# gersteinlab/LESSeq

Hardware: AMD Instinct MI355X
Metric: MRF reads/sec through count+solve (higher is better)
Workload: dtype int32 coordinates / u64 counters (count), f64 (EM); 1 GPU; BASELINE configs[2]: 100M synthetic 100bp reads over 50k mixed events (SE/RI/A5SS/A3SS/MXE/AFE/ALE/T3), 24 chromosomes; events=50000

## Files before the change

include/lesseq_hip_dev.h:

```cpp
#ifndef LESSEQ_HIP_DEV_H
#define LESSEQ_HIP_DEV_H

#include <stdint.h>
#include "lesseq_hip.h"

#ifdef __cplusplus
extern "C" {
#endif

int lsq_debug_counters(lsq_ctx *c, unsigned long long *out16);
int lsq_debug_wg_trace(lsq_ctx *c, unsigned long long *out, unsigned long long cap, unsigned long long *n, unsigned long long *n_workers);

int lsq_debug_slot_offsets(lsq_ctx *c, int method, unsigned long long *out, unsigned long long n);
int lsq_debug_plan_shares(const unsigned long long *slot_off, const unsigned char *packed, const unsigned long long *n1, const unsigned long long *n2,
                          const unsigned *look1, const unsigned *look2, unsigned long long n_buckets, unsigned long long grid,
                          const double *costs4, int weighted, int snap, unsigned long long *cuts);
int lsq_debug_offsets(lsq_ctx *c, int method, int which, unsigned long long *out, unsigned long long cap, unsigned long long *n);

int lsq_debug_set_em_order(lsq_ctx *c, const uint32_t *order, unsigned n_small_places, unsigned n_places);

int lsq_debug_last_em_launch(lsq_ctx *c, unsigned out[8]);

int lsq_debug_stream_read_rate(lsq_ctx *c, unsigned long long bytes, double *gb_per_s);

int lsq_debug_throw(int kind);

int lsq_debug_last_parse_paths(const lsq_ctx *c, unsigned *tiles_handed, unsigned *lines_listed, unsigned *all_slow);

int lsq_debug_bgzf_inflate(lsq_ctx *c, const void *bytes, uint64_t len, void *out, uint64_t cap, uint64_t *n);

int lsq_debug_bgzf_crc32(lsq_ctx *c, const void *bytes, uint64_t len, uint32_t *crc, uint64_t cap, uint64_t *n);

// ... 9 lines not shown
```

lesseq_amd/csrc/lsq_count.hip:

```cpp
#include "lsq_device.hpp"
#include <hip/hip_ext.h>

namespace {

#ifndef LSQ_COUNT_BLOCK
#define LSQ_COUNT_BLOCK 256
#endif
constexpr int COUNT_BLOCK = LSQ_COUNT_BLOCK;
constexpr unsigned long long BASES_MASK = (1ull << 40) - 1;

#ifdef LSQ_DEV
#define ABL(args, bits) ((((args).ablate) & (bits)) != 0u)
#else
#define ABL(args, bits) false
#endif


struct CountArgs {
	const BucketDesc *buckets;
	const unsigned char *images;
	const TieRec *ties;
	const unsigned char *strand_rank;
	const char *read_names; const unsigned long long *read_name_off;
	const char *gene_names; const unsigned *gene_name_off;
	unsigned n_buckets;
	unsigned ablate;
	unsigned tables_lds_bytes;
	const void *p1; const unsigned char *p1_strand; const unsigned *p1_line;
	const void *p2; const unsigned char *p2_strand; const unsigned *p2_line;
	unsigned compact;
	const unsigned *pn_blk_off; const unsigned *pn_nblk; const int2 *pn_se; const unsigned char *pn_strand; const unsigned *pn_line; const unsigned *pn_bucket;
	const unsigned long long *p1_off, *p2_off, *pn_off, *slot_off;
	const lsq::VisitRec *visits;
	const unsigned *wg_first;
	const unsigned long long *wg_cut;
	const lsq::WgPlan *wg_plan;
	unsigned long long *wg_trace;
	unsigned long long total_slots;
	unsigned long long n_pn;
	unsigned n_workers;
	unsigned long long *cnt, *bases;
	struct ExcEntry *exc;
	unsigned *exc_count;
	unsigned exc_cap;
	unsigned long long *dbg;
// ... 604 lines not shown
	};
	if (ww0 < ww1) fetch(ww0);
	for (unsigned wt = ww0; wt < ww1; wt += WAVES * TILE) {
		uint4 cur[SW];
#pragma unroll
		for (int k = 0; k < SW; ++k) cur[k] = nxt[k];
		if (wt + WAVES * TILE < ww1) fetch(wt + WAVES * TILE);
		do_step(cur, wt);
	}
	if (R.live() && !ABL(A, 32u)) walk_parked<NB>(C, R, true);
}


template <int NR>
__device__ inline void stream_pool1_compact(FastCtx &C, const uint4 *bins, const uint4 *cells, const uint4 *cellx, const unsigned n_cells, const BucketDesc &d,
                                            const CountArgs &A, uint4 *queue, const void *pool, const unsigned long long g0, const unsigned long long g1) {
	static_assert(NR == 4 || NR == 8, "one or two 16-byte words of four compact records");
	static_assert((unsigned)NR <= P1_GROUP_PAD, "a lane's records of a step lie in one cell group");
	constexpr int CW = NR / 4;
	constexpr unsigned TILE = 64u * NR;
	C.pool = 0u;
	C.slot0 = g0;
	global_words src = (global_words)pool;
	const unsigned lane = threadIdx.x & 63u, wave = (unsigned)__builtin_amdgcn_readfirstlane((int)(threadIdx.x >> 6));
	const unsigned long long R0 = g0 & ~(unsigned long long)(NR - 1);
	const unsigned n = (unsigned)(g1 - R0), first_rel = (unsigned)(g0 - R0), n_rel = (unsigned)(g1 - g0);
	const unsigned last_word = (n - 1u) >> 2;
	const int base = d.lo - lsq::COMPACT_BIAS;
	uint4 nxt[CW];
	auto fetch = [&](const unsigned t) {
#pragma unroll
// ... 37 lines not shown
#pragma unroll
			for (int j = 0; j < NR; ++j) {
				const unsigned len = rec[j] >> lsq::COMPACT_OFF_BITS;
				const int e = (int)(rec[j] & lsq::COMPACT_OFF_MASK) + (int)len;
				unsigned p = len | (min(len, 1u) << 24);
				if (!decltype(whole_step)::value) {
					const unsigned idx = t + lane * (unsigned)NR + (unsigned)j;
					p = (idx < n && idx - first_rel < n_rel) ? p : 0u;
				}
				accN += p;
				accA += e <= e1 ? p : 0u;
				if (!decltype(one_threshold)::value) accL += e <= e2 ? p : 0u;
			}
			if (decltype(one_threshold)::value) accL = accA;
		};
		if (__all(e1 == e2) && !ABL(A, 8388608u)) { if (interior) decide(std::true_type{}, std::true_type{}); else decide(std::false_type{}, std::true_type{}); }
		else { if (interior) decide(std::true_type{}, std::false_type{}); else decide(std::false_type{}, std::false_type{}); }
		const unsigned s1 = cx.x & 0xFFFFu, s2 = cx.x >> 16;
		if (!ABL(A, (1u | 16384u))) {
			const unsigned acc2 = both ? accL : accL - accA;
			if (accA && s1 != CELL_NONE) atomicAdd(&C.hist[s1], ((unsigned long long)(accA >> 24) << 40) | (accA & 0xFFFFFFu));
			if (acc2 && s2 != CELL_NONE) atomicAdd(&C.hist[s2], ((unsigned long long)(acc2 >> 24) << 40) | (acc2 & 0xFFFFFFu));
		} else asm volatile("" ::"v"(accA), "v"(accL));
		const bool lane_open = (accN >> 24) != ((both ? accA : accL) >> 24);
		if (ABL(A, 256u)) {
			const bool any_open = __any(lane_open);
			if (lane == 0) { atomicAdd(&A.dbg[12], 1ull); atomicAdd(&A.dbg[11], any_open ? 1ull : 0ull); }
		}
		if (__any(lane_open) && !ABL(A, 17u | 524288u)) {
#pragma unroll
			for (int h = 0; h < NR; h += 2) {
// ... 16 lines not shown
					if (ABL(A, 256u) && op) { atomicAdd(&A.dbg[5 + (has ? (both ? 2 : 1) : 0)], 1ull); atomicAdd(&A.dbg[0], 1ull); }
				}
				R.push2(open, lane, en[0], en[1]);
				if (R.live() >= 64u) {
					if (!ABL(A, 32u)) walk_parked<1, false>(C, R, false, base);
					else R.head = R.tail;
				}
			}
		}
	}
	if (R.live() && !ABL(A, 32u)) walk_parked<1, false>(C, R, true, base);
}

template <int NR>
__device__ inline void stream_pool2_compact(FastCtx &C, const uint4 *bins, const uint4 *cells, const uint4 *cellx, const unsigned n_cells, const BucketDesc &d,
                                            const CountArgs &A, uint4 *queue, const void *pool, const unsigned long long g0, const unsigned long long g1) {
	static_assert((NR == 2 || NR == 4 || NR == 8) && (unsigned)NR <= P2_GROUP_PAD, "whole 16-byte words of two compact records, inside one junction group");
	constexpr int CW = NR / 2;
	constexpr unsigned TILE = 64u * NR;
	C.pool = 1u;
	C.slot0 = g0;
	global_words src = (global_words)pool;
	const unsigned lane = threadIdx.x & 63u, wave = (unsigned)__builtin_amdgcn_readfirstlane((int)(threadIdx.x >> 6));
	const unsigned long long R0 = g0 & ~(unsigned long long)(NR - 1);
	const unsigned n = (unsigned)(g1 - R0), first_rel = (unsigned)(g0 - R0), n_rel = (unsigned)(g1 - g0);
	const unsigned last_word = (n - 1u) >> 1;
	const int base = d.lo - lsq::COMPACT_BIAS;
	uint4 nxt[CW];
	auto fetch = [&](const unsigned t) {
#pragma unroll
		for (int cq = 0; cq < CW; ++cq) {
// ... 76 lines not shown
		};
		bool none[NR];
#pragma unroll
		for (int j = 0; j < NR; ++j) none[j] = false;
		if (any_plain) {
#pragma unroll
			for (int j = 0; j < NR; ++j) none[j] = !junction && nothing(ra[j], rb[j]);
		}
		bool park[NR];
		park[0] = in0 && len1 != 0u && !(J || Jb || S || drop || none[0]) && !ABL(A, 17u | 1048576u);
		if (ABL(A, 256u) && park[0]) atomicAdd(&A.dbg[8 + (v1 ? 1 : 0)], 1ull);
		unsigned nA = (in0 && J && slotA != CELL_NONE) ? 1u : 0u, sA = nA ? total : 0u, nB = (in0 && Jb && slotB != CELL_NONE) ? 1u : 0u, sB = nB ? total : 0u;
		const int lim = junction ? end2 - rd.y : -1, limb = junction ? end2b - rd.y : -1;
		bool any_park = park[0];
		const bool any_b = __any(limb > lim) || ABL(A, 8388608u);
#pragma unroll
		for (int j = 1; j < NR; ++j) {
			const unsigned l1 = ra[j] >> lsq::COMPACT_OFF_BITS, l2 = rb[j] >> lsq::COMPACT_OFF_BITS;
			const int reach = (int)(rb[j] & lsq::COMPACT_OFF_MASK) + (int)l2;
			bool in = l1 != 0u;
			if (!interior) { const unsigned idx = idx0 + (unsigned)j; in = in && idx < n && idx - first_rel < n_rel; }
			const bool sameA = in && reach <= lim;
			bool sameB = false;
			const bool cA = sameA && slotA != CELL_NONE;
			nA += cA ? 1u : 0u; sA += cA ? l1 + l2 : 0u;
			if (any_b) {
				sameB = in && reach > lim && reach <= limb;
				const bool cB = sameB && slotB != CELL_NONE;
				nB += cB ? 1u : 0u; sB += cB ? l1 + l2 : 0u;
			}
			park[j] = in && !(sameA || sameB || none[j]) && !ABL(A, 17u | 1048576u | 2097152u);
			if (ABL(A, 256u) && park[j]) atomicAdd(&A.dbg[junction ? 14 : 13], 1ull);
			any_park = any_park || park[j];
		}
		if (!ABL(A, 1u)) {
			if (addS) atomicAdd(&C.hist[sa], (1ull << 40) | len1);
			if (nA) atomicAdd(&C.hist[slotA], ((unsigned long long)nA << 40) | sA);
			if (nB) atomicAdd(&C.hist[slotB], ((unsigned long long)nB << 40) | sB);
		} else asm volatile("" ::"v"(nA), "v"(sA), "v"(nB), "v"(sB));
		if (__any(any_park)) {
			const unsigned hint0 = v1 ? (cx1.w | PARK_ONE_EVENT) : evf;
#pragma unroll
			for (int h = 0; h < NR; h += 2) {
				const uint4 qa = make_uint4(ra[h], rb[h], h == 0 ? hint0 : PARK_EVENT_UNKNOWN, rel0 + (unsigned)h);
				const uint4 qb = make_uint4(ra[h + 1], rb[h + 1], PARK_EVENT_UNKNOWN, rel0 + (unsigned)h + 1u);
				if (ABL(A, 256u)) atomicAdd(&A.dbg[1], (park[h] ? 1ull : 0ull) + (park[h + 1] ? 1ull : 0ull));
				R.push2((park[h] ? 1u : 0u) | (park[h + 1] ? 2u : 0u), lane, qa, qb);
				if (R.live() >= 64u) {
					if (!ABL(A, 32u)) walk_parked<2, true>(C, R, false, base);
// ... 102 lines not shown
	const unsigned long long s_begin = plan->s_begin, s_end = plan->s_end;
	if (s_begin >= s_end) return;
	if (ABL(A, 4096u)) return;
	const_visit vr = &plan->first;
	unsigned b = vr->b;
	bool first_visit = true;
	while (b < A.n_buckets) {
		const unsigned long long bs = vr->bs;
		if (bs >= s_end) break;
		BucketDesc d;
		d.img_off = vr->d.img_off; d.img_bytes = vr->d.img_bytes; d.n_events = vr->d.n_events; d.n_bins = vr->d.n_bins; d.lo = vr->d.lo; d.shift = vr->d.shift;
		d.ev_off = vr->d.ev_off; d.seg_off = vr->d.seg_off; d.iso_off = vr->d.iso_off; d.hist_off = vr->d.hist_off; d.n_cls = vr->d.n_cls; d.cls_base = vr->d.cls_base;
		d.ev_base = vr->d.ev_base; d.chrom_id = vr->d.chrom_id; d.kind = vr->d.kind; d.hi = vr->d.hi;
		const unsigned long long be = vr->be, p1o = vr->p1o, n1 = vr->p1n, p2o = vr->p2o, n2 = vr->p2n;
		const unsigned next = vr->next;
		unsigned char *buf = lds;
		if (!first_visit) __syncthreads();
		first_visit = false;
		{
			global_words src = (global_words)(A.images + d.img_off);
			uint4 *dst = reinterpret_cast<uint4 *>(buf);
			for (unsigned i = tid; i < d.img_bytes / 16; i += COUNT_BLOCK) { const u32x4 t = src[i]; dst[i] = make_uint4(t.x, t.y, t.z, t.w); }
			unsigned long long *h = reinterpret_cast<unsigned long long *>(buf + d.hist_off);
			for (unsigned i = tid; i < HIST_REPLICAS * (d.n_cls | 1u); i += COUNT_BLOCK) h[i] = 0;
		}
		__syncthreads();
		if (ABL(A, 8192u)) return;
		const uint4 *bins = reinterpret_cast<const uint4 *>(buf);
		const uint4 *cells = reinterpret_cast<const uint4 *>(buf + d.seg_off);
		const unsigned n_cells = d.iso_off & 0xFFFFu;
		const uint4 *cellx = reinterpret_cast<const uint4 *>(buf + d.seg_off + 16u * (d.iso_off >> 16));
		FastCtx C;
		C.bins = bins; C.lo = d.lo; C.shift = d.shift; C.n_bins = d.n_bins;
		C.recs = reinterpret_cast<const uint4 *>(buf + d.ev_off);
		C.hist = reinterpret_cast<unsigned long long *>(buf + d.hist_off) + (tid & (HIST_REPLICAS - 1u)) * (d.n_cls | 1u);
		C.n_events = d.n_events; C.bucket = b;
		C.slot0 = 0; C.pool = 0;
		C.exc = A.exc; C.exc_count = A.exc_count; C.exc_cap = A.exc_cap; C.ablate = A.ablate; C.dbg = A.dbg;
		C.trace = (ABL(A, 4194304u) && A.wg_trace) ? A.wg_trace + 4u * blockIdx.x : nullptr;
		const unsigned long long l0 = (s_begin > bs ? s_begin : bs) - bs;
		const unsigned long long l1 = (s_end < be ? s_end : be) - bs;
		if (l0 < n1 && !ABL(A, 1024u)) {
			if constexpr (COMPACT) stream_pool1_compact<2 * P1W>(C, bins, cells, cellx, n_cells, d, A, wave_queue, A.p1, p1o + l0, p1o + (l1 < n1 ? l1 : n1));
			else stream_pool_wide<2>(C, bins, cells, cellx, n_cells, d, A, wave_queue, reinterpret_cast<const uint4 *>(A.p1), p1o + l0, p1o + (l1 < n1 ? l1 : n1));
		}
		if (l1 > n1 && l0 < n1 + n2 && !ABL(A, 2048u)) {
			const unsigned long long q0 = p2o + ((l0 > n1 ? l0 : n1) - n1), q1 = p2o + ((l1 < n1 + n2 ? l1 : n1 + n2) - n1);
			if constexpr (COMPACT) stream_pool2_compact<(P1W == 4 ? LSQ_P2_COMPACT_WORDS_W5 : LSQ_P2_COMPACT_WORDS)>(C, bins, cells, cellx, n_cells, d, A, wave_queue, A.p2, q0, q1);
			else stream_pool_wide<1>(C, bins, cells, cellx, n_cells, d, A, wave_queue, reinterpret_cast<const uint4 *>(A.p2), q0, q1);
		}
		__syncthreads();
		for (unsigned i = tid; i < d.n_cls; i += COUNT_BLOCK) {
			const unsigned long long *h0 = reinterpret_cast<const unsigned long long *>(buf + d.hist_off) + i;
			unsigned long long v = 0;
#pragma unroll
			for (unsigned r = 0; r < HIST_REPLICAS; ++r) v += h0[r * (d.n_cls | 1u)];
			if (v && !ABL(A, 4u)) {
				atomicAdd(&A.cnt[d.cls_base + i], v >> 40);
				atomicAdd(&A.bases[d.cls_base + i], v & BASES_MASK);
			}
		}
		if (be >= s_end) break;
		b = next;
// ... 297 lines not shown
				if ((rc = mr.wg_plan.upload(plan.data(), plan.size(), st))) return rc;
				HIP_TRY(hipStreamSynchronize(st));
			}
			HIP_TRY(hipStreamSynchronize(st));
			mr.wg_grid = grid;
		}
		CountArgs A{};
		A.buckets = c->buckets.p; A.images = c->images.p; A.ties = c->ties.p; A.strand_rank = c->strand_rank.p;
		A.wg_first = mr.wg_first.p; A.wg_cut = mr.wg_cut.p; A.wg_plan = mr.wg_plan.p; A.visits = mr.visits.p;
		A.read_names = mr.named ? mr.names.p : nullptr; A.read_name_off = mr.named ? mr.name_off.p : nullptr;
		A.gene_names = c->gene_names.p; A.gene_name_off = c->gene_name_off.p;
		A.n_buckets = (unsigned)E.buckets.size();
		A.tables_lds_bytes = tables_bytes;
		A.ablate = c->dev_ablate;
		A.compact = mr.compact ? 1u : 0u;
		A.p1 = mr.p1.p; A.p1_strand = mr.p1_strand.p; A.p1_line = mr.p1_line.p;
		A.p2 = mr.p2.p; A.p2_strand = mr.p2_strand.p; A.p2_line = mr.p2_line.p;
		A.pn_blk_off = mr.pn_blk_off.p; A.pn_nblk = mr.pn_nblk.p; A.pn_se = reinterpret_cast<const int2 *>(mr.pn_se.p);
		A.pn_strand = mr.pn_strand.p; A.pn_line = mr.pn_line.p; A.pn_bucket = mr.pn_bucket.p;
		A.p1_off = mr.p1_off.p; A.p2_off = mr.p2_off.p; A.pn_off = mr.pn_off.p; A.slot_off = mr.slot_off.p;
		A.total_slots = mr.total_slots;
		A.cnt = c->cnt.p + (size_t)m * n_cls; A.bases = c->bases.p + (size_t)m * n_cls;
		A.exc = mr.exc.p + (size_t)set * mr.exc_cap; A.exc_count = c->exc_count.p + 2 * m; A.exc_cap = (unsigned)mr.exc_cap;
		A.dbg = c->dbg.p; A.bar = c->dbg.p + 16 + m;
		A.wg_trace = nullptr;
		const unsigned long long n_pn = mr.pn_strand.n;
		A.n_pn = n_pn;
		const unsigned workers_per_cu = 2;
		A.n_workers = (unsigned)std::min<unsigned long long>((n_pn + COUNT_BLOCK - 1) / COUNT_BLOCK, (unsigned long long)c->n_cu * workers_per_cu);
#ifdef LSQ_DEV
// ... 136 lines not shown
```

lesseq_amd/csrc/lsq_device.hip:

```cpp
#include "lsq_device.hpp"
#include <chrono>
#include <thread>

namespace lsq {

int upload_strand_ranks(lsq_ctx *c) {
	const auto &names = c->E->strands.names;
	if (names.size() > 256) return fail(LSQ_E_RANGE, "more than 256 distinct strand strings");
	std::vector<int> order(names.size());
	std::iota(order.begin(), order.end(), 0);
	std::sort(order.begin(), order.end(), [&](int a, int b) { return names[a] < names[b]; });
	std::vector<uint8_t> rank(256, 0);
	for (size_t r = 0; r < order.size(); ++r) rank[order[r]] = (uint8_t)r;
	int rc = c->strand_rank.upload(rank.data(), 256, c->stream);
	if (rc) return rc;
	HIP_TRY(hipStreamSynchronize(c->stream));
	return LSQ_OK;
}

static hipError_t wait_for_stream(hipStream_t s) {
	const auto t0 = std::chrono::steady_clock::now();
	for (;;) {
		const hipError_t e = hipStreamQuery(s);
		if (e != hipErrorNotReady) return e;
// ... 817 lines not shown
	} else if (n == "sam_min_mapq") {
		if (!(value >= 0 && value <= 256)) return fail(LSQ_E_ARG, "sam_min_mapq must lie in 0..256");
		c->opt_sam_min_mapq = (unsigned)value;
	} else if (n == "bam_verify") {
		if (!(value == 0 || value == 1)) return fail(LSQ_E_ARG, "bam_verify must be 0 or 1");
		c->opt_bam_verify = value == 1;
	} else if (n == "compact_pools") {
		c->opt_compact_pools = value != 0;
	} else if (n == "workgroups_per_cu") {
		if (!(value >= -1 && value <= 32)) return fail(LSQ_E_ARG, "workgroups_per_cu must lie in -1..32 (-1 = automatic, 0 = as many as fit)");
		c->opt_wg_per_cu = (int)value;
		c->occ_lds_bytes = 0;
	} else if (n == "reads_per_look") {
		if (!(value == 0 || value == 4 || value == 8)) return fail(LSQ_E_ARG, "reads_per_look must be 0 (automatic), 4 or 8");
		c->opt_reads_per_look = (int)value;
	} else if (n == "count_streams") {
		{ int rc = sync_all(c); if (rc) return rc; }
		c->opt_two_count_streams = value >= 2;
	} else if (n == "em_flat_min_events") {
		if (!(value >= 0 && value <= 4e9)) return fail(LSQ_E_ARG, "em_flat_min_events must lie in 0..4e9");
		c->em.opt_flat_min = (unsigned)value;
	} else if (n == "em_closed_form") {
		{ int rc = sync_all(c); if (rc) return rc; }
		c->em.opt_closed = value != 0;
	} else if (n == "em_quad_cap") {
		if (value < 0 || value > 1e6) return fail(LSQ_E_ARG, "em_quad_cap out of range");
		c->em.opt_quad_cap = (unsigned)value;
	} else if (n == "em_regroup") {
		c->em.opt_regroup = value != 0;
		for (EmLane &l : c->em.lane) l.order_valid = false;
// ... 41 lines not shown
```

lesseq_amd/csrc/lsq_device.hpp:

```cpp
#pragma once
#include <hip/hip_runtime.h>

#include <algorithm>
#include <cmath>
#include <cstring>
#include <memory>
#include <numeric>
#include <string>
#include <thread>
#include <type_traits>
#include <vector>

#include "lsq_internal.hpp"

using namespace lsq;

#define HIP_TRY(expr)                                                                          \
	do {                                                                                       \
		hipError_t _e = (expr);                                                                \
		if (_e != hipSuccess) return fail(LSQ_E_DEVICE, "%s: %s", #expr, hipGetErrorString(_e)); \
	} while (0)


#ifndef LSQ_P1_PAD
// ... 60 lines not shown
}

struct RouteChrom {
	unsigned loc_first, loc_nb;
	int loc_base;
	unsigned cov0, cov1, clu0, clu1;
	unsigned pad;
};
static_assert(sizeof(RouteChrom) == 32, "RouteChrom is staged in LDS as two 16-byte words");

struct VisitRec {
	BucketDesc d;
	unsigned long long bs, be;
	unsigned long long p1o, p1n, p2o, p2n;
	unsigned b, next;
	unsigned pad[2];
};
static_assert(sizeof(VisitRec) == 128, "VisitRec is read as 32 dwords");
struct WgPlan {
	unsigned long long s_begin, s_end;
	VisitRec first;
};
static_assert(sizeof(WgPlan) == 144, "WgPlan layout");

struct IngestPass {
	const char *name = nullptr;
	hipEvent_t ev[2] = {nullptr, nullptr};
	unsigned long long bytes = 0;
	float ms = 0;
	bool clocked = false;
};
// ... 76 lines not shown
	hipStream_t stream_em2[2] = {nullptr, nullptr};
	hipStream_t stream_count2[2] = {nullptr, nullptr};
	bool opt_two_count_streams = true;
	int opt_wg_per_cu = -1;
	hipEvent_t ev_counted2[2] = {nullptr, nullptr}, ev_mark2[2] = {nullptr, nullptr};
	bool mark_recorded2[2] = {false, false};
	int flip = 0;
	size_t counters_per_set = 0;
	hipEvent_t ev0 = nullptr, ev1 = nullptr, ev2 = nullptr, ev3 = nullptr;
	hipEvent_t evt0 = nullptr, evt1 = nullptr;
	hipEvent_t evf0[LSQ_MAX_METHODS] = {}, evf1[LSQ_MAX_METHODS] = {};
	int fast_launched = 0;
	int occ_p1w = 0;
	int opt_reads_per_look = 0;
	unsigned last_reads_per_look = 4, last_wg_per_cu = 0;
	unsigned occ_lds_bytes = 0; int occ_blocks = 0;
	bool time_events = false;
	bool count_timed = false, solve_timed = false;
	lsq_events *E = nullptr;
	DevBuf<BucketDesc> buckets;
	DevBuf<uint8_t> images, strand_rank, dK;
	DevBuf<TieRec> ties;
	DevBuf<uint32_t> cls_base, iso_base, gene_name_off;
	DevBuf<char> gene_names;
	DevBuf<uint32_t> pack_cls, pack_iso, pack_ev;
	EmState em;
	DevBuf<double> G, theta2[2], logll2[2];
	DevBuf<uint32_t> iters2[2];
	DevBuf<uint8_t> flags2[2];
	DevView<double> theta, logll;
// ... 84 lines not shown
```

lesseq_amd/csrc/lsq_ingest.hip:

```cpp
#include "lsq_ingest.hpp"
#include "lsq_text.hpp"

namespace {

struct IngestRaw {
	unsigned long long n_reads;
	const unsigned long long *blk_off;
	const unsigned *line_no;
	const int *blk_start, *blk_end;
	const unsigned short *blk_chrom;
	const unsigned char *blk_strand;
};

#ifndef LSQ_RAW_WAVES
#define LSQ_RAW_WAVES 8
#endif
template <bool STRANDED, class... Lib>
__global__ void __launch_bounds__(256) __attribute__((amdgpu_waves_per_eu(LSQ_RAW_WAVES))) lsq_route_raw_kernel(RouteTables T, IngestRaw R, RouteOut O, Lib... lib_arg) {
	__shared__ RouteChrom chrom_lds[ROUTE_CHROM_LDS];
	const RouteChrom *chroms = route_stage_chroms(T, chrom_lds);
	const unsigned long long gsz = (unsigned long long)gridDim.x * blockDim.x;
	LocProbe P;
	P.chrom = -1; P.bin = 0;
	if constexpr (!STRANDED) {
// ... 266 lines not shown
	else reinterpret_cast<int4 *>(out)[at] = r;
}

struct PlaceArgs {
	const uint4 *pieces;
	const unsigned long long *part_off1, *part_off2;
	const uint4 *part1, *part2;
	const unsigned *fine1, *fine2;
	const unsigned long long *off1, *off2;
	unsigned *cur1, *cur2;
	const BucketDesc *buckets;
	const unsigned *cell_base, *jg_base, *jgroup_base;
	unsigned B, compact;
	void *p1; unsigned char *p1_strand; unsigned *p1_line;
	void *p2; unsigned char *p2_strand; unsigned *p2_line;
};

__global__ void __launch_bounds__(256) lsq_group_place_kernel(PlaceArgs A) {
	extern __shared__ __align__(16) unsigned char glds[];
	unsigned *cur = reinterpret_cast<unsigned *>(glds);
	const uint4 pc = A.pieces[blockIdx.x];
	const unsigned pool = pc.x >= A.B ? 1u : 0u, b = pc.x - pool * A.B;
	const BucketDesc &d = A.buckets[b];
	const unsigned n_cells = d.kind == 1u ? (d.iso_off & 0xFFFFu) : 0u;
	const unsigned n_groups = pool ? (A.jg_base[b + 1] - A.jg_base[b]) + n_cells + 1u : n_cells + 1u;
	const unsigned gbase = pool ? A.jgroup_base[b] : A.cell_base[b];
	const unsigned long long first = (pool ? A.part_off2[b] : A.part_off1[b]) + pc.y;
	const unsigned *fine = (pool ? A.fine2 : A.fine1) + first;
	unsigned *goff = cur + n_groups;
	const unsigned long long *off = pool ? A.off2 : A.off1;
	const unsigned long long off0 = off[gbase];
	for (unsigned q = threadIdx.x; q < n_groups; q += 256u) { cur[q] = 0; goff[q] = (unsigned)(off[gbase + q] - off0); }
	__syncthreads();
	if (!pc.w) {
		for (unsigned r = threadIdx.x; r < pc.z; r += 256u) atomicAdd(&cur[fine[r] - gbase], 1u);
		__syncthreads();
		unsigned *gcur = pool ? A.cur2 : A.cur1;
		for (unsigned q = threadIdx.x; q < n_groups; q += 256u) { const unsigned c = cur[q]; cur[q] = c ? atomicAdd(&gcur[gbase + q], c) : 0u; }
		__syncthreads();
	}
	const int base = d.lo - lsq::COMPACT_BIAS;
	for (unsigned r0 = threadIdx.x; r0 < pc.z; r0 += 1024u) {
		unsigned g[4]; uint4 v[4], x[4]; bool on[4];
#pragma unroll
		for (int u = 0; u < 4; ++u) {
			const unsigned r = r0 + 256u * (unsigned)u;
			on[u] = r < pc.z;
			g[u] = on[u] ? fine[r] - gbase : 0u;
			if (!pool) { v[u] = on[u] ? A.part1[first + r] : make_uint4(0, 0, 0, 0); x[u] = v[u]; }
			else { v[u] = on[u] ? A.part2[2ull * (first + r)] : make_uint4(0, 0, 0, 0); x[u] = on[u] ? A.part2[2ull * (first + r) + 1] : make_uint4(0, 0, 0, 0); }
		}
#pragma unroll
		for (int u = 0; u < 4; ++u) {
			if (!on[u]) continue;
			const unsigned long long w = off0 + goff[g[u]] + atomicAdd(&cur[g[u]], 1u);
			if (!pool) {
				const int2 rec = make_int2((int)v[u].x, (int)v[u].y);
				if (A.compact) pool_store<true>(A.p1, w, rec, base); else pool_store<false>(A.p1, w, rec, base);
				A.p1_strand[w] = (unsigned char)v[u].w; A.p1_line[w] = v[u].z;
			} else {
				const int4 rec = make_int4((int)v[u].x, (int)v[u].y, (int)v[u].z, (int)v[u].w);
				if (A.compact) pool_store<true>(A.p2, w, rec, base); else pool_store<false>(A.p2, w, rec, base);
				A.p2_strand[w] = (unsigned char)x[u].y; A.p2_line[w] = x[u].x;
			}
		}
	}
}

struct NbOut {
	const uint4 *ent; const int2 *blk; unsigned long long n_ent;
	const unsigned long long *pn_off, *pnb_off;
	unsigned *curn, *curnb;
	unsigned *pn_blk_off, *pn_nblk, *pn_line, *pn_bucket; unsigned char *pn_strand; int2 *pn_se;
	const unsigned *line_no; unsigned long long first_line;
};
__global__ void __launch_bounds__(256) lsq_ingest_nblock_kernel(NbOut O) {
	const unsigned long long gsz = (unsigned long long)gridDim.x * blockDim.x;
	for (unsigned long long t = (unsigned long long)blockIdx.x * blockDim.x + threadIdx.x; t < O.n_ent; t += gsz) {
		const uint4 en = O.ent[t];
		const unsigned i = en.x, b = en.y, n = en.z & 0xFFu, strand = en.z >> 8;
// ... 75 lines not shown
	const unsigned long long n = F.n;
	if (B >= ROUTE_NO_BUCKET) return fail(LSQ_E_RANGE, "more than 2^22 buckets");
	if (n > 0xFFFFFFF0ull) return fail(LSQ_E_RANGE, "more than 2^32 reads in one file");
	hipStream_t st = c->stream;
	int rc;
	if ((rc = ensure_lanes(c))) return rc;
	HIP_TRY(hipStreamSynchronize(c->stream_em2[0]));
	HIP_TRY(hipStreamSynchronize(c->stream_em2[1]));
	HIP_TRY(hipStreamSynchronize(c->stream_count2[0]));
	HIP_TRY(hipStreamSynchronize(c->stream_count2[1]));
	const size_t FC = c->n_cell_groups;
	const size_t FJ = c->n_junction_groups;
	const size_t n_cnt = 10 * (size_t)B + 3 * (FC + FJ);
	const size_t n_tot = 8 + ROUTE_LIB_WORD0 + (E.stranded() ? 8 * (size_t)ROUTE_LIB_SLOTS : 0);
	std::vector<unsigned long long> lib_places(E.stranded() ? 8 * (size_t)ROUTE_LIB_SLOTS : 0);
	DevBuf<unsigned> d_key, d_cnt, d_fine1, d_fine2;
	DevBuf<int4> d_rec;
	DevBuf<unsigned long long> d_tot, d_part_off1, d_part_off2, d_piece_off, d_off1, d_off2;
	DevBuf<uint4> d_nb_ent, d_part1, d_part2, d_pieces;
	DevBuf<int2> d_nb_blk;
	ScanScratch SS;
	if ((rc = d_key.alloc(n)) || (rc = d_rec.alloc(n)) || (rc = d_cnt.alloc(n_cnt)) || (rc = d_tot.alloc(n_tot)) || (rc = d_part_off1.alloc(B + 1)) || (rc = d_part_off2.alloc(B + 1)) ||
	    (rc = d_piece_off.alloc(2 * (size_t)B + 1)) || (rc = d_off1.alloc(FC + 1)) || (rc = d_off2.alloc(FJ + 1)) || (rc = SS.reserve(std::max<size_t>(std::max(FC, FJ), 2 * (size_t)B)))) return rc;
	unsigned *part_cnt = d_cnt.p, *part_cur = part_cnt + 2 * (size_t)B, *piece_cnt = part_cur + 2 * (size_t)B;
	unsigned *cntn = piece_cnt + 2 * (size_t)B, *cntnb = cntn + B, *curn = cntnb + B, *curnb = curn + B;
	unsigned *cnt1 = curnb + B, *cnt2 = cnt1 + FC, *cur1 = cnt2 + FJ, *cur2 = cur1 + FC, *park1 = cur2 + FJ, *park2 = park1 + FC;
	if ((rc = mr.p1_off.alloc(B + 1)) || (rc = mr.p2_off.alloc(B + 1)) || (rc = mr.pn_off.alloc(B + 1)) || (rc = mr.pnb_off.alloc(B + 1)) || (rc = mr.slot_off.alloc(B + 1))) return rc;
	const RouteTables T = route_tables(c);
	const size_t part_lds = 8 * (size_t)B;
	const bool part_in_lds = part_lds <= 128 * 1024 && getenv("LSQ_PART_NO_LDS") == nullptr;
	size_t img_max = 16, jg_max = 0, groups_max = 1;
	for (unsigned b = 0; b < B; ++b) {
		const BucketDesc &d = E.buckets[b];
		const size_t n_cells = d.kind == 1u ? (d.iso_off & 0xFFFFu) : 0u, n_jg = E.jg_base[b + 1] - E.jg_base[b];
		if (d.kind == 1u) img_max = std::max<size_t>(img_max, (d.img_bytes + 15u) & ~15u);
		jg_max = std::max(jg_max, n_jg);
		groups_max = std::max(groups_max, n_jg + n_cells + 1);
	}
// ... 103 lines not shown
	}
	SW.mark("ingest: partition + group launches");
	HIP_TRY(hipMemcpyAsync(&psum[0], mr.p1_off.p + B, 8, hipMemcpyDeviceToHost, st));
	HIP_TRY(hipMemcpyAsync(&psum[1], mr.p2_off.p + B, 8, hipMemcpyDeviceToHost, st));
	HIP_TRY(hipStreamSynchronize(st));
	SW.mark("ingest: partition + groups");
	const size_t n1 = (size_t)psum[0], n2 = (size_t)psum[1];
	mr.compact = compact != 0;
	mr.n1_reads = tot[4]; mr.n2_reads = tot[5];
	if ((rc = mr.p1.alloc(mr.compact ? ((n1 + 3) & ~(size_t)3) : 2 * n1)) || (rc = mr.p1_strand.alloc(n1)) || (rc = mr.p1_line.alloc(n1))) return rc;
	if ((rc = mr.p2.alloc(mr.compact ? 2 * ((n2 + 1) & ~(size_t)1) : 4 * n2)) || (rc = mr.p2_strand.alloc(n2)) || (rc = mr.p2_line.alloc(n2))) return rc;
	if ((rc = mr.pn_se.alloc(2 * nnb)) || (rc = mr.pn_blk_off.alloc(nn)) || (rc = mr.pn_nblk.alloc(nn)) || (rc = mr.pn_strand.alloc(nn)) ||
	    (rc = mr.pn_line.alloc(nn)) || (rc = mr.pn_bucket.alloc(nn))) return rc;
	{
		StageClock k(c, st, "group_place");
		if (n_pieces) {
			PlaceArgs P{};
			P.pieces = d_pieces.p; P.part_off1 = d_part_off1.p; P.part_off2 = d_part_off2.p; P.part1 = d_part1.p; P.part2 = d_part2.p;
			P.fine1 = d_fine1.p; P.fine2 = d_fine2.p; P.off1 = d_off1.p; P.off2 = d_off2.p; P.cur1 = cur1; P.cur2 = cur2;
			P.buckets = c->buckets.p; P.cell_base = c->cell_base.p; P.jg_base = c->jg_base.p; P.jgroup_base = c->jgroup_base.p; P.B = B; P.compact = compact;
			P.p1 = mr.p1.p; P.p1_strand = mr.p1_strand.p; P.p1_line = mr.p1_line.p; P.p2 = mr.p2.p; P.p2_strand = mr.p2_strand.p; P.p2_line = mr.p2_line.p;
			hipLaunchKernelGGL(lsq_group_place_kernel, dim3((unsigned)n_pieces), dim3(256), place_lds, st, P);
		}
		if (FC + FJ) {
			const unsigned pgrid = (unsigned)std::min<size_t>((FC + FJ) / 256 + 1, (size_t)c->n_cu * 8);
			hipLaunchKernelGGL(lsq_ingest_pad_kernel, dim3(pgrid), dim3(256), 0, st, c->buckets.p, c->cell_base.p, c->jgroup_base.p, B, (unsigned)FC, (unsigned)FJ,
			                   (const unsigned *)cnt1, (const unsigned long long *)d_off1.p, (const unsigned *)cnt2, (const unsigned long long *)d_off2.p, c->images.p,
			                   (void *)mr.p1.p, (void *)mr.p2.p, compact, mr.p1_strand.p, mr.p1_line.p, mr.p2_strand.p, mr.p2_line.p);
		}
		if (nn) {
			NbOut N{};
			N.ent = d_nb_ent.p; N.blk = d_nb_blk.p; N.n_ent = nb_tot[0]; N.pn_off = mr.pn_off.p; N.pnb_off = mr.pnb_off.p; N.curn = curn; N.curnb = curnb;
			N.pn_blk_off = mr.pn_blk_off.p; N.pn_nblk = mr.pn_nblk.p; N.pn_line = mr.pn_line.p; N.pn_bucket = mr.pn_bucket.p; N.pn_strand = mr.pn_strand.p;
			N.pn_se = reinterpret_cast<int2 *>(mr.pn_se.p); N.line_no = F.line_no; N.first_line = F.first_line;
			const unsigned ngrid = (unsigned)std::min<unsigned long long>((nb_tot[0] + 255) / 256, (unsigned long long)c->n_cu * 16);
			hipLaunchKernelGGL(lsq_ingest_nblock_kernel, dim3(ngrid), dim3(256), 0, st, N);
// ... 15 lines not shown
		mr.lib_report[q] = 0;
		for (size_t k = 0; k < lib_places.size(); k += 8) mr.lib_report[q] += lib_places[k + q];
	}
	mr.n_retained_blocks = tot[1] + nb_tot[1];
	mr.total_slots = n1 + n2 + nn;
	mr.wg_grid = 0;
	{
		std::vector<unsigned long long> so(B + 1, 0), o1(B + 1, 0), o2(B + 1, 0), f1(FC + 1, 0), f2(FJ + 1, 0);
		std::vector<unsigned> park(FC + FJ + 1, 0);
		HIP_TRY(hipMemcpyAsync(so.data(), mr.slot_off.p, (B + 1) * sizeof(unsigned long long), hipMemcpyDeviceToHost, st));
		HIP_TRY(hipMemcpyAsync(o1.data(), mr.p1_off.p, (B + 1) * sizeof(unsigned long long), hipMemcpyDeviceToHost, st));
		HIP_TRY(hipMemcpyAsync(o2.data(), mr.p2_off.p, (B + 1) * sizeof(unsigned long long), hipMemcpyDeviceToHost, st));
		HIP_TRY(hipMemcpyAsync(f1.data(), d_off1.p, (FC + 1) * sizeof(unsigned long long), hipMemcpyDeviceToHost, st));
		HIP_TRY(hipMemcpyAsync(f2.data(), d_off2.p, (FJ + 1) * sizeof(unsigned long long), hipMemcpyDeviceToHost, st));
		if (FC + FJ) HIP_TRY(hipMemcpyAsync(park.data(), park1, (FC + FJ) * sizeof(unsigned), hipMemcpyDeviceToHost, st));
		HIP_TRY(hipStreamSynchronize(st));
		SW.mark("ingest: place + read-back");
		stages_collect(c);
		unsigned long long mx = 0;
		for (unsigned b = 0; b < B; ++b) mx = std::max(mx, so[b + 1] - so[b]);
		mr.slot_off_host = so;
		mr.skew = (B && mr.total_slots) ? (double)mx * (double)B / (double)mr.total_slots : 1.0;
		{
			mr.plan_n1.resize(B); mr.plan_n2.resize(B); mr.plan_park1.assign(B, 0); mr.plan_park2.assign(B, 0);
			mr.plan_seg_x.clear(); mr.plan_seg_kind.clear(); mr.plan_seg_looks.clear(); mr.plan_seg_first.assign(B + 1, 0);
			size_t g1 = 0, g2 = 0;
			for (unsigned b = 0; b < B; ++b) {
				const unsigned n_cg = (E.buckets[b].kind == 1 ? (E.buckets[b].iso_off & 0xFFFFu) : 0u) + 1u, n_jg = (E.jg_base[b + 1] - E.jg_base[b]) + n_cg;
				const unsigned long long n1 = o1[b + 1] - o1[b], n2 = o2[b + 1] - o2[b], ns = so[b + 1] - so[b];
				mr.plan_n1[b] = n1; mr.plan_n2[b] = n2;
// ... 15 lines not shown
				g1 += n_cg; g2 += n_jg;
			}
			mr.plan_seg_first[B] = (unsigned)mr.plan_seg_kind.size();
			mr.plan_seg_x.push_back(B ? so[B] : 0);
		}
		std::vector<VisitRec> vis(B + 1);
		mr.next_packed_host.assign(B + 1, B);
		memset(vis.data(), 0, vis.size() * sizeof(VisitRec));
		unsigned next = B;
		for (unsigned b = B; b-- > 0;) {
			VisitRec &v = vis[b];
			v.d = E.buckets[b];
			v.bs = so[b]; v.be = so[b + 1];
			v.p1o = o1[b]; v.p1n = o1[b + 1] - o1[b]; v.p2o = o2[b]; v.p2n = o2[b + 1] - o2[b];
			v.b = b; v.next = next;
			if (E.buckets[b].kind == 1u && so[b + 1] > so[b]) next = b;
			mr.next_packed_host[b] = next;
		}
		vis[B].b = B; vis[B].next = B; vis[B].bs = vis[B].be = mr.total_slots;
		if ((rc = mr.visits.upload(vis.data(), vis.size(), st))) return rc;
		mr.visits_host = vis;
		HIP_TRY(hipStreamSynchronize(st));
	}
	mr.present = true;
	c->counted = c->solved = false;
	SW.mark("ingest: plan, visit records");
	return LSQ_OK;
}

namespace {
// ... 114 lines not shown
```

lesseq_amd/csrc/lsq_replay.hip:

```cpp
#include "lsq_device.hpp"
#include <atomic>


namespace {

struct HostRead {
	int start, end;
	unsigned line;
	unsigned matched;
	unsigned short cls;
	unsigned char strand;
};

struct HostWalk {
	long long pos = 0; int it = 0; bool found = false; uint64_t mask = 0; long long matched = 0;
	bool block(const lsq::Event &e, long long a, long long b) {
		while (it < e.N) {
			const long long sx = e.seg_s[(size_t)it], sy = e.seg_e[(size_t)it];
			if (!(sx < b)) break;
			pos = std::max(pos, sx);
			if (a >= pos && a < sy) {
				if (found && a > pos) break;
				found = true;
				mask |= 1ull << it;
// ... 429 lines not shown
	if (!mr.present) return fail(LSQ_E_STATE, "no reads uploaded for method %d", method);
	for (int q = 0; q < 6; ++q) out[q] = 0;
	for (size_t b = 0; b < E.buckets.size(); ++b) {
		const lsq::BucketDesc &d = E.buckets[b];
		BucketReads R;
		{ int rc = fetch_bucket(mr, b, d.lo, R); if (rc) return rc; }
		const lsq::Cell *cells = d.kind == 1 ? reinterpret_cast<const lsq::Cell *>(E.images.data() + d.img_off + d.seg_off) : nullptr;
		const unsigned n_cells = d.kind == 1 ? (d.iso_off & 0xFFFFu) : 0u;
		auto cell_of = [&](int p) -> long {
			for (unsigned q = 0; q < n_cells; ++q) if (cells[q].lo <= p && p < cells[q].hi) return (long)q;
			return -1;
		};
		const size_t n1 = R.p1_line.size(), n2 = R.p2_line.size();
		if ((n1 % P1_GROUP_PAD) || (n2 % P2_GROUP_PAD)) return fail(LSQ_E_STATE, "bucket %zu: pool slices of %zu and %zu records are not whole groups of %u / %u", b, n1, n2, P1_GROUP_PAD, P2_GROUP_PAD);
		out[0] += n1; out[3] += n2;
		for (size_t q = 0; q < n1; q += P1_GROUP_PAD) {
			long first = -2;
			bool mixed = false;
			for (size_t k = q; k < q + P1_GROUP_PAD; ++k) {
				const int s = R.p1[2 * k], e = R.p1[2 * k + 1];
				if (s == e) { ++out[1]; continue; }
				const long cl = cell_of(s);
				if (first == -2) first = cl; else if (cl != first) mixed = true;
			}
			if (mixed) ++out[2];
		}
		const uint64_t *k0 = E.jg_keys.data() + E.jg_base[b], *k1 = E.jg_keys.data() + E.jg_base[b + 1];
		auto group_of = [&](const int32_t *r) -> long {
			const long cl = cell_of(r[0]);
			if (cl < 0 || (r[1] != cells[cl].e1 && r[1] != cells[cl].e2)) return -1;
// ... 12 lines not shown
				const bool eb = rb[0] == rb[1];
				out[4] += eb ? 1u : 0u;
				if (ea) bad = bad || !eb;
				else if (ga >= 0 && !eb && group_of(rb) != ga) bad = true;
				else if (ga < 0 && !eb && (group_of(rb) >= 0 || cell_of(rb[0]) != cell_of(ra[0]))) bad = true;
			}
			if (bad) ++out[5];
		}
	}
	if (out[0] - out[1] != mr.n1_reads || out[3] - out[4] != mr.n2_reads)
		return fail(LSQ_E_STATE, "the pools hold %llu + %llu reads, the ingest counted %llu + %llu", out[0] - out[1], out[3] - out[4],
		            (unsigned long long)mr.n1_reads, (unsigned long long)mr.n2_reads);
	return LSQ_OK;
} LSQ_API_CATCH

}
```

Before: 749.8 billion reads/s.

## Add uniform read-length fast path to compact pool counting

At ingest the place kernel now records, per bucket, the minimum and maximum read length for one-block reads and the minimum and maximum total length for two-block reads. When a bucket's lengths are all equal, the visit record carries that length. The counting kernels then replace per-record length extraction and summation with compare-only counting multiplied by the common length. The goal is to cut ALU work in the hot streaming loops, at the cost of extra atomics in the place kernel and a small host read-back.

```diff
diff --git a/include/lesseq_hip_dev.h b/include/lesseq_hip_dev.h
--- a/include/lesseq_hip_dev.h
+++ b/include/lesseq_hip_dev.h
@@ -16,6 +16,9 @@
                           const unsigned *look1, const unsigned *look2, unsigned long long n_buckets, unsigned long long grid,
                           const double *costs4, int weighted, int snap, unsigned long long *cuts);
 int lsq_debug_offsets(lsq_ctx *c, int method, int which, unsigned long long *out, unsigned long long cap, unsigned long long *n);
+
+int lsq_debug_uniform_lengths(lsq_ctx *c, int method, unsigned *len1, unsigned *tot2, unsigned long long cap, unsigned long long *n);
+int lsq_debug_check_pool_layout(lsq_ctx *c, int method, unsigned long long *out);
 
 int lsq_debug_set_em_order(lsq_ctx *c, const uint32_t *order, unsigned n_small_places, unsigned n_places);
 
diff --git a/lesseq_amd/csrc/lsq_count.hip b/lesseq_amd/csrc/lsq_count.hip
--- a/lesseq_amd/csrc/lsq_count.hip
+++ b/lesseq_amd/csrc/lsq_count.hip
@@ -29,6 +29,7 @@
 	const void *p1; const unsigned char *p1_strand; const unsigned *p1_line;
 	const void *p2; const unsigned char *p2_strand; const unsigned *p2_line;
 	unsigned compact;
+	unsigned uniform_len;
 	const unsigned *pn_blk_off; const unsigned *pn_nblk; const int2 *pn_se; const unsigned char *pn_strand; const unsigned *pn_line; const unsigned *pn_bucket;
 	const unsigned long long *p1_off, *p2_off, *pn_off, *slot_off;
 	const lsq::VisitRec *visits;
@@ -663,7 +664,7 @@
 
 template <int NR>
 __device__ inline void stream_pool1_compact(FastCtx &C, const uint4 *bins, const uint4 *cells, const uint4 *cellx, const unsigned n_cells, const BucketDesc &d,
-                                            const CountArgs &A, uint4 *queue, const void *pool, const unsigned long long g0, const unsigned long long g1) {
+                                            const CountArgs &A, uint4 *queue, const void *pool, const unsigned long long g0, const unsigned long long g1, const unsigned ulen) {
 	static_assert(NR == 4 || NR == 8, "one or two 16-byte words of four compact records");
 	static_assert((unsigned)NR <= P1_GROUP_PAD, "a lane's records of a step lie in one cell group");
 	constexpr int CW = NR / 4;
@@ -731,7 +732,30 @@
 			}
 			if (decltype(one_threshold)::value) accL = accA;
 		};
-		if (__all(e1 == e2) && !ABL(A, 8388608u)) { if (interior) decide(std::true_type{}, std::true_type{}); else decide(std::false_type{}, std::true_type{}); }
+		auto decide_uniform = [&](auto one_threshold) {
+			const unsigned K = ulen << lsq::COMPACT_OFF_BITS, off_end = 1u << lsq::COMPACT_OFF_BITS;
+			unsigned tA = e1 < (int)ulen ? 0u : min((unsigned)e1 - ulen + 1u, off_end);
+			unsigned tL = e2 < (int)ulen ? 0u : min((unsigned)e2 - ulen + 1u, off_end);
+			asm volatile("" : "+v"(tA));
+			if (!decltype(one_threshold)::value) asm volatile("" : "+v"(tL));
+			unsigned nN = 0, nA = 0, nL = 0;
+#pragma unroll
+			for (int j = 0; j < NR; ++j) {
+				const unsigned u = rec[j] - K;
+				nN += u < off_end ? 1u : 0u;
+				nA += u < tA ? 1u : 0u;
+				if (!decltype(one_threshold)::value) nL += u < tL ? 1u : 0u;
+			}
+			const unsigned ul = ulen & (lsq::COMPACT_MAX_LEN - 1u);
+			asm volatile("" : "+v"(nN), "+v"(nA));
+			if (!decltype(one_threshold)::value) asm volatile("" : "+v"(nL));
+			accN = (nN & 15u) * ul + (nN << 24);
+			accA = (nA & 15u) * ul + (nA << 24);
+			accL = decltype(one_threshold)::value ? accA : (nL & 15u) * ul + (nL << 24);
+		};
+		const bool one_threshold = __all(e1 == e2) && !ABL(A, 8388608u);
+		if (interior && ulen != 0u) { if (one_threshold) decide_uniform(std::true_type{}); else decide_uniform(std::false_type{}); }
+		else if (one_threshold) { if (interior) decide(std::true_type{}, std::true_type{}); else decide(std::false_type{}, std::true_type{}); }
 		else { if (interior) decide(std::true_type{}, std::false_type{}); else decide(std::false_type{}, std::false_type{}); }
 		const unsigned s1 = cx.x & 0xFFFFu, s2 = cx.x >> 16;
 		if (!ABL(A, (1u | 16384u))) {
@@ -778,7 +802,7 @@
 
 template <int NR>
 __device__ inline void stream_pool2_compact(FastCtx &C, const uint4 *bins, const uint4 *cells, const uint4 *cellx, const unsigned n_cells, const BucketDesc &d,
-                                            const CountArgs &A, uint4 *queue, const void *pool, const unsigned long long g0, const unsigned long long g1) {
+                                            const CountArgs &A, uint4 *queue, const void *pool, const unsigned long long g0, const unsigned long long g1, const unsigned utot) {
 	static_assert((NR == 2 || NR == 4 || NR == 8) && (unsigned)NR <= P2_GROUP_PAD, "whole 16-byte words of two compact records, inside one junction group");
 	constexpr int CW = NR / 2;
 	constexpr unsigned TILE = 64u * NR;
@@ -885,6 +909,7 @@
 		const int lim = junction ? end2 - rd.y : -1, limb = junction ? end2b - rd.y : -1;
 		bool any_park = park[0];
 		const bool any_b = __any(limb > lim) || ABL(A, 8388608u);
+		auto followers = [&](auto per_record_sums) {
 #pragma unroll
 		for (int j = 1; j < NR; ++j) {
 			const unsigned l1 = ra[j] >> lsq::COMPACT_OFF_BITS, l2 = rb[j] >> lsq::COMPACT_OFF_BITS;
@@ -894,16 +919,25 @@
 			const bool sameA = in && reach <= lim;
 			bool sameB = false;
 			const bool cA = sameA && slotA != CELL_NONE;
-			nA += cA ? 1u : 0u; sA += cA ? l1 + l2 : 0u;
+			nA += cA ? 1u : 0u;
+			if (decltype(per_record_sums)::value) sA += cA ? l1 + l2 : 0u;
 			if (any_b) {
 				sameB = in && reach > lim && reach <= limb;
 				const bool cB = sameB && slotB != CELL_NONE;
-				nB += cB ? 1u : 0u; sB += cB ? l1 + l2 : 0u;
+				nB += cB ? 1u : 0u;
+				if (decltype(per_record_sums)::value) sB += cB ? l1 + l2 : 0u;
 			}
 			park[j] = in && !(sameA || sameB || none[j]) && !ABL(A, 17u | 1048576u | 2097152u);
 			if (ABL(A, 256u) && park[j]) atomicAdd(&A.dbg[junction ? 14 : 13], 1ull);
 			any_park = any_park || park[j];
 		}
+		};
+		if (utot != 0u) {
+			followers(std::false_type{});
+			asm volatile("" : "+v"(nA));
+			sA = (nA & 15u) * (utot & 2047u);
+			if (any_b) { asm volatile("" : "+v"(nB)); sB = (nB & 15u) * (utot & 2047u); }
+		} else followers(std::true_type{});
 		if (!ABL(A, 1u)) {
 			if (addS) atomicAdd(&C.hist[sa], (1ull << 40) | len1);
 			if (nA) atomicAdd(&C.hist[slotA], ((unsigned long long)nA << 40) | sA);
@@ -1036,6 +1070,9 @@
 		d.ev_base = vr->d.ev_base; d.chrom_id = vr->d.chrom_id; d.kind = vr->d.kind; d.hi = vr->d.hi;
 		const unsigned long long be = vr->be, p1o = vr->p1o, n1 = vr->p1n, p2o = vr->p2o, n2 = vr->p2n;
 		const unsigned next = vr->next;
+		const unsigned len1 = A.uniform_len ? vr->len1 : 0u;
+		const unsigned tot2 = A.uniform_len ? vr->tot2 : 0u;
+		(void)len1; (void)tot2;
 		unsigned char *buf = lds;
 		if (!first_visit) __syncthreads();
 		first_visit = false;
@@ -1063,12 +1100,12 @@
 		const unsigned long long l0 = (s_begin > bs ? s_begin : bs) - bs;
 		const unsigned long long l1 = (s_end < be ? s_end : be) - bs;
 		if (l0 < n1 && !ABL(A, 1024u)) {
-			if constexpr (COMPACT) stream_pool1_compact<2 * P1W>(C, bins, cells, cellx, n_cells, d, A, wave_queue, A.p1, p1o + l0, p1o + (l1 < n1 ? l1 : n1));
+			if constexpr (COMPACT) stream_pool1_compact<2 * P1W>(C, bins, cells, cellx, n_cells, d, A, wave_queue, A.p1, p1o + l0, p1o + (l1 < n1 ? l1 : n1), len1);
 			else stream_pool_wide<2>(C, bins, cells, cellx, n_cells, d, A, wave_queue, reinterpret_cast<const uint4 *>(A.p1), p1o + l0, p1o + (l1 < n1 ? l1 : n1));
 		}
 		if (l1 > n1 && l0 < n1 + n2 && !ABL(A, 2048u)) {
 			const unsigned long long q0 = p2o + ((l0 > n1 ? l0 : n1) - n1), q1 = p2o + ((l1 < n1 + n2 ? l1 : n1 + n2) - n1);
-			if constexpr (COMPACT) stream_pool2_compact<(P1W == 4 ? LSQ_P2_COMPACT_WORDS_W5 : LSQ_P2_COMPACT_WORDS)>(C, bins, cells, cellx, n_cells, d, A, wave_queue, A.p2, q0, q1);
+			if constexpr (COMPACT) stream_pool2_compact<(P1W == 4 ? LSQ_P2_COMPACT_WORDS_W5 : LSQ_P2_COMPACT_WORDS)>(C, bins, cells, cellx, n_cells, d, A, wave_queue, A.p2, q0, q1, tot2);
 			else stream_pool_wide<1>(C, bins, cells, cellx, n_cells, d, A, wave_queue, reinterpret_cast<const uint4 *>(A.p2), q0, q1);
 		}
 		__syncthreads();
@@ -1396,6 +1433,7 @@
 		A.tables_lds_bytes = tables_bytes;
 		A.ablate = c->dev_ablate;
 		A.compact = mr.compact ? 1u : 0u;
+		A.uniform_len = c->opt_uniform_len ? 1u : 0u;
 		A.p1 = mr.p1.p; A.p1_strand = mr.p1_strand.p; A.p1_line = mr.p1_line.p;
 		A.p2 = mr.p2.p; A.p2_strand = mr.p2_strand.p; A.p2_line = mr.p2_line.p;
 		A.pn_blk_off = mr.pn_blk_off.p; A.pn_nblk = mr.pn_nblk.p; A.pn_se = reinterpret_cast<const int2 *>(mr.pn_se.p);
diff --git a/lesseq_amd/csrc/lsq_device.hip b/lesseq_amd/csrc/lsq_device.hip
--- a/lesseq_amd/csrc/lsq_device.hip
+++ b/lesseq_amd/csrc/lsq_device.hip
@@ -855,6 +855,9 @@
 	} else if (n == "reads_per_look") {
 		if (!(value == 0 || value == 4 || value == 8)) return fail(LSQ_E_ARG, "reads_per_look must be 0 (automatic), 4 or 8");
 		c->opt_reads_per_look = (int)value;
+	} else if (n == "uniform_length_path") {
+		if (!(value == 0 || value == 1)) return fail(LSQ_E_ARG, "uniform_length_path must be 0 or 1");
+		c->opt_uniform_len = value == 1;
 	} else if (n == "count_streams") {
 		{ int rc = sync_all(c); if (rc) return rc; }
 		c->opt_two_count_streams = value >= 2;
diff --git a/lesseq_amd/csrc/lsq_device.hpp b/lesseq_amd/csrc/lsq_device.hpp
--- a/lesseq_amd/csrc/lsq_device.hpp
+++ b/lesseq_amd/csrc/lsq_device.hpp
@@ -98,7 +98,7 @@
 	unsigned long long bs, be;
 	unsigned long long p1o, p1n, p2o, p2n;
 	unsigned b, next;
-	unsigned pad[2];
+	unsigned len1, tot2;
 };
 static_assert(sizeof(VisitRec) == 128, "VisitRec is read as 32 dwords");
 struct WgPlan {
@@ -205,6 +205,7 @@
 	int occ_p1w = 0;
 	int opt_reads_per_look = 0;
 	unsigned last_reads_per_look = 4, last_wg_per_cu = 0;
+	bool opt_uniform_len = true;
 	unsigned occ_lds_bytes = 0; int occ_blocks = 0;
 	bool time_events = false;
 	bool count_timed = false, solve_timed = false;
diff --git a/lesseq_amd/csrc/lsq_ingest.hip b/lesseq_amd/csrc/lsq_ingest.hip
--- a/lesseq_amd/csrc/lsq_ingest.hip
+++ b/lesseq_amd/csrc/lsq_ingest.hip
@@ -304,6 +304,7 @@
 	unsigned B, compact;
 	void *p1; unsigned char *p1_strand; unsigned *p1_line;
 	void *p2; unsigned char *p2_strand; unsigned *p2_line;
+	unsigned *len_min1, *len_max1, *tot_min2, *tot_max2;
 };
 
 __global__ void __launch_bounds__(256) lsq_group_place_kernel(PlaceArgs A) {
@@ -321,6 +322,9 @@
 	const unsigned long long *off = pool ? A.off2 : A.off1;
 	const unsigned long long off0 = off[gbase];
 	for (unsigned q = threadIdx.x; q < n_groups; q += 256u) { cur[q] = 0; goff[q] = (unsigned)(off[gbase + q] - off0); }
+	__shared__ unsigned span[2];
+	if (threadIdx.x == 0) { span[0] = 0xFFFFFFFFu; span[1] = 0u; }
+	unsigned len_lo = 0xFFFFFFFFu, len_hi = 0u;
 	__syncthreads();
 	if (!pc.w) {
 		for (unsigned r = threadIdx.x; r < pc.z; r += 256u) atomicAdd(&cur[fine[r] - gbase], 1u);
@@ -344,6 +348,8 @@
 		for (int u = 0; u < 4; ++u) {
 			if (!on[u]) continue;
 			const unsigned long long w = off0 + goff[g[u]] + atomicAdd(&cur[g[u]], 1u);
+			const unsigned len = !pool ? v[u].y - v[u].x : (v[u].y - v[u].x) + (v[u].w - v[u].z);
+			len_lo = min(len_lo, len); len_hi = max(len_hi, len);
 			if (!pool) {
 				const int2 rec = make_int2((int)v[u].x, (int)v[u].y);
 				if (A.compact) pool_store<true>(A.p1, w, rec, base); else pool_store<false>(A.p1, w, rec, base);
@@ -354,6 +360,12 @@
 				A.p2_strand[w] = (unsigned char)x[u].y; A.p2_line[w] = x[u].x;
 			}
 		}
+	}
+	if (len_lo <= len_hi) { atomicMin(&span[0], len_lo); atomicMax(&span[1], len_hi); }
+	__syncthreads();
+	if (threadIdx.x == 0 && span[0] <= span[1]) {
+		atomicMin(&(pool ? A.tot_min2 : A.len_min1)[b], span[0]);
+		atomicMax(&(pool ? A.tot_max2 : A.len_max1)[b], span[1]);
 	}
 }
 
@@ -459,14 +471,14 @@
 	const size_t n_cnt = 10 * (size_t)B + 3 * (FC + FJ);
 	const size_t n_tot = 8 + ROUTE_LIB_WORD0 + (E.stranded() ? 8 * (size_t)ROUTE_LIB_SLOTS : 0);
 	std::vector<unsigned long long> lib_places(E.stranded() ? 8 * (size_t)ROUTE_LIB_SLOTS : 0);
-	DevBuf<unsigned> d_key, d_cnt, d_fine1, d_fine2;
+	DevBuf<unsigned> d_key, d_cnt, d_fine1, d_fine2, d_len;
 	DevBuf<int4> d_rec;
 	DevBuf<unsigned long long> d_tot, d_part_off1, d_part_off2, d_piece_off, d_off1, d_off2;
 	DevBuf<uint4> d_nb_ent, d_part1, d_part2, d_pieces;
 	DevBuf<int2> d_nb_blk;
 	ScanScratch SS;
 	if ((rc = d_key.alloc(n)) || (rc = d_rec.alloc(n)) || (rc = d_cnt.alloc(n_cnt)) || (rc = d_tot.alloc(n_tot)) || (rc = d_part_off1.alloc(B + 1)) || (rc = d_part_off2.alloc(B + 1)) ||
-	    (rc = d_piece_off.alloc(2 * (size_t)B + 1)) || (rc = d_off1.alloc(FC + 1)) || (rc = d_off2.alloc(FJ + 1)) || (rc = SS.reserve(std::max<size_t>(std::max(FC, FJ), 2 * (size_t)B)))) return rc;
+	    (rc = d_piece_off.alloc(2 * (size_t)B + 1)) || (rc = d_len.alloc(4 * (size_t)B)) || (rc = d_off1.alloc(FC + 1)) || (rc = d_off2.alloc(FJ + 1)) || (rc = SS.reserve(std::max<size_t>(std::max(FC, FJ), 2 * (size_t)B)))) return rc;
 	unsigned *part_cnt = d_cnt.p, *part_cur = part_cnt + 2 * (size_t)B, *piece_cnt = part_cur + 2 * (size_t)B;
 	unsigned *cntn = piece_cnt + 2 * (size_t)B, *cntnb = cntn + B, *curn = cntnb + B, *curnb = curn + B;
 	unsigned *cnt1 = curnb + B, *cnt2 = cnt1 + FC, *cur1 = cnt2 + FJ, *cur2 = cur1 + FC, *park1 = cur2 + FJ, *park2 = park1 + FC;
@@ -600,12 +612,17 @@
 	    (rc = mr.pn_line.alloc(nn)) || (rc = mr.pn_bucket.alloc(nn))) return rc;
 	{
 		StageClock k(c, st, "group_place");
+		if (B) {
+			HIP_TRY(hipMemsetAsync(d_len.p, 0xFF, 2 * (size_t)B * sizeof(unsigned), st));
+			HIP_TRY(hipMemsetAsync(d_len.p + 2 * (size_t)B, 0, 2 * (size_t)B * sizeof(unsigned), st));
+		}
 		if (n_pieces) {
 			PlaceArgs P{};
 			P.pieces = d_pieces.p; P.part_off1 = d_part_off1.p; P.part_off2 = d_part_off2.p; P.part1 = d_part1.p; P.part2 = d_part2.p;
 			P.fine1 = d_fine1.p; P.fine2 = d_fine2.p; P.off1 = d_off1.p; P.off2 = d_off2.p; P.cur1 = cur1; P.cur2 = cur2;
 			P.buckets = c->buckets.p; P.cell_base = c->cell_base.p; P.jg_base = c->jg_base.p; P.jgroup_base = c->jgroup_base.p; P.B = B; P.compact = compact;
 			P.p1 = mr.p1.p; P.p1_strand = mr.p1_strand.p; P.p1_line = mr.p1_line.p; P.p2 = mr.p2.p; P.p2_strand = mr.p2_strand.p; P.p2_line = mr.p2_line.p;
+			P.len_min1 = d_len.p; P.tot_min2 = d_len.p + B; P.len_max1 = d_len.p + 2 * (size_t)B; P.tot_max2 = d_len.p + 3 * (size_t)B;
 			hipLaunchKernelGGL(lsq_group_place_kernel, dim3((unsigned)n_pieces), dim3(256), place_lds, st, P);
 		}
 		if (FC + FJ) {
@@ -651,6 +668,8 @@
 		HIP_TRY(hipMemcpyAsync(f1.data(), d_off1.p, (FC + 1) * sizeof(unsigned long long), hipMemcpyDeviceToHost, st));
 		HIP_TRY(hipMemcpyAsync(f2.data(), d_off2.p, (FJ + 1) * sizeof(unsigned long long), hipMemcpyDeviceToHost, st));
 		if (FC + FJ) HIP_TRY(hipMemcpyAsync(park.data(), park1, (FC + FJ) * sizeof(unsigned), hipMemcpyDeviceToHost, st));
+		std::vector<unsigned> span(4 * (size_t)B + 1, 0);
+		if (B) HIP_TRY(hipMemcpyAsync(span.data(), d_len.p, 4 * (size_t)B * sizeof(unsigned), hipMemcpyDeviceToHost, st));
 		HIP_TRY(hipStreamSynchronize(st));
 		SW.mark("ingest: place + read-back");
 		stages_collect(c);
@@ -696,6 +715,9 @@
 			v.bs = so[b]; v.be = so[b + 1];
 			v.p1o = o1[b]; v.p1n = o1[b + 1] - o1[b]; v.p2o = o2[b]; v.p2n = o2[b + 1] - o2[b];
 			v.b = b; v.next = next;
+			const unsigned lo1 = span[b], lo2 = span[B + b], hi1 = span[2 * (size_t)B + b], hi2 = span[3 * (size_t)B + b];
+			v.len1 = (mr.compact && lo1 == hi1) ? lo1 : 0u;
+			v.tot2 = (mr.compact && lo2 == hi2) ? lo2 : 0u;
 			if (E.buckets[b].kind == 1u && so[b + 1] > so[b]) next = b;
 			mr.next_packed_host[b] = next;
 		}
diff --git a/lesseq_amd/csrc/lsq_replay.hip b/lesseq_amd/csrc/lsq_replay.hip
--- a/lesseq_amd/csrc/lsq_replay.hip
+++ b/lesseq_amd/csrc/lsq_replay.hip
@@ -467,6 +467,26 @@
 		const size_t n1 = R.p1_line.size(), n2 = R.p2_line.size();
 		if ((n1 % P1_GROUP_PAD) || (n2 % P2_GROUP_PAD)) return fail(LSQ_E_STATE, "bucket %zu: pool slices of %zu and %zu records are not whole groups of %u / %u", b, n1, n2, P1_GROUP_PAD, P2_GROUP_PAD);
 		out[0] += n1; out[3] += n2;
+		{
+			unsigned lo[2] = {0xFFFFFFFFu, 0xFFFFFFFFu}, hi[2] = {0u, 0u};
+			for (size_t k = 0; k < n1; ++k) {
+				const unsigned len = (unsigned)(R.p1[2 * k + 1] - R.p1[2 * k]);
+				if (len) { lo[0] = std::min(lo[0], len); hi[0] = std::max(hi[0], len); }
+			}
+			for (size_t k = 0; k < n2; ++k) {
+				const int32_t *r = &R.p2[4 * k];
+				const unsigned tot = (unsigned)(r[1] - r[0]) + (unsigned)(r[3] - r[2]);
+				if (r[1] != r[0]) { lo[1] = std::min(lo[1], tot); hi[1] = std::max(hi[1], tot); }
+			}
+			if (b >= mr.visits_host.size()) return fail(LSQ_E_STATE, "bucket %zu has no visit record", b);
+			const unsigned named[2] = {mr.visits_host[b].len1, mr.visits_host[b].tot2};
+			for (int p = 0; p < 2; ++p) {
+				const unsigned want = (mr.compact && lo[p] == hi[p]) ? lo[p] : 0u;
+				if (named[p] != want)
+					return fail(LSQ_E_STATE, "bucket %zu: the visit record names %u as the common %s of its %s-block reads, which run from %u to %u (%s records)", b, named[p],
+					            p ? "total" : "length", p ? "two" : "one", lo[p] <= hi[p] ? lo[p] : 0u, hi[p], mr.compact ? "compact" : "wide");
+			}
+		}
 		for (size_t q = 0; q < n1; q += P1_GROUP_PAD) {
 			long first = -2;
 			bool mixed = false;
@@ -509,4 +529,15 @@
 	return LSQ_OK;
 } LSQ_API_CATCH
 
-}
+int lsq_debug_uniform_lengths(lsq_ctx *c, int method, unsigned *len1, unsigned *tot2, unsigned long long cap, unsigned long long *n) LSQ_API_TRY {
+	if (!c || !c->E || !len1 || !tot2 || !n || method < 0 || method >= c->E->n_methods) return fail(LSQ_E_ARG, "bad argument");
+	const lsq::MethodReads &mr = c->reads[method];
+	if (!mr.present) return fail(LSQ_E_STATE, "no reads uploaded for method %d", method);
+	const size_t B = c->E->buckets.size();
+	*n = B;
+	if (cap < B || mr.visits_host.size() < B) return fail(LSQ_E_RANGE, "%zu buckets", B);
+	for (size_t b = 0; b < B; ++b) { len1[b] = mr.visits_host[b].len1; tot2[b] = mr.visits_host[b].tot2; }
+	return LSQ_OK;
+} LSQ_API_CATCH
+
+}
```

Measured after the change: 743.6 billion reads/s. About the same (-0.8%).
